# rgrover/cloud-haskell-paxos

Measured on AMD Instinct MI355X. Metric: Paxos instances decided/sec (node), higher is better.
Workload: dtype int32

## Files before the change

### cloud-haskell-paxos_amd/csrc/paxos_ev.h

```cpp
#pragma once
#include <hip/hip_runtime.h>
#include <stdint.h>

#include <type_traits>

#include "../../include/paxos_batch.h"
#include "ev_layouts.h"
#include "paxos_device.h"

namespace pxb {
namespace ev {

#ifndef PXB_EV_SL_RH
#define PXB_EV_SL_RH 1
#endif
#ifndef PXB_EV_LG_RH
#define PXB_EV_LG_RH 0
#endif
#ifndef PXB_EV_STORE_BACK
#define PXB_EV_STORE_BACK 1
#endif
#ifndef PXB_EV_PQ_CAP
#define PXB_EV_PQ_CAP 4
#endif
// ... 93 lines not shown
#else
#define PXB_EV_PROBE(b, c) ((void)0)
#endif

__host__ __device__ __forceinline__ uint32_t u24(uint32_t x) { return x & 0xFFFFFFu; }
template <uint32_t C>
__host__ __device__ __forceinline__ uint32_t mulc(uint32_t x) { return ((C & (C - 1u)) == 0u) ? x * C : u24(x) * C; }
__host__ __device__ __forceinline__ uint32_t ctz32(uint32_t x) { return x ? (uint32_t)__builtin_ctz(x) : 32u; }
__host__ __device__ __forceinline__ uint32_t popc32(uint32_t x) { return (uint32_t)__builtin_popcount(x); }
__host__ __device__ __forceinline__ uint32_t nbits32(uint32_t x) { return x ? 32u - (uint32_t)__builtin_clz(x) : 0u; }

__host__ __device__ __forceinline__ uint32_t window_of(const EvParams& kp, const uint4& w, uint32_t crash_m1) {
  uint32_t c0 = 0, c1 = 0;
  if (w.x <= crash_m1) {
    c0 = mulhi_n(w.y, kp.crash_start_max + 1u);
    c1 = c0 + 1u + mulhi_n(w.z, kp.crash_len_max);
  }
  c0 = c0 < 4096u ? c0 : 4096u;
  c1 = c1 < 4096u ? c1 : 4096u;
  return c0 | (c1 << 16);
}

__host__ __device__ __forceinline__ bool crash_of(const EvParams& kp, uint64_t inst, uint32_t& crash_m1) {
  crash_m1 = kp.crash_m1;
  if (!(kp.cfg & EV_CFG_RANDOMIZE)) return (kp.cfg & EV_CFG_CRASHY) != 0u;
  const uint4 w = philox((uint32_t)inst, (uint32_t)(inst >> 32), 0u, 4u << 24, kp.k0, kp.k1);
  const uint64_t ct = ev_threshold(mulhi_n(w.w, kp.crash_ppm + 1u));
  crash_m1 = (uint32_t)(ct - 1ull);
  return ct != 0ull;
}

__host__ __device__ __forceinline__ uint32_t window_word(const EvParams& kp, uint64_t inst, uint32_t a, bool crashy,
                                                         uint32_t crash_m1) {
  if (!crashy) return 0u;
  return window_of(kp, philox((uint32_t)inst, (uint32_t)(inst >> 32), 0u, (3u << 24) | a, kp.k0, kp.k1), crash_m1);
}

struct EvOut {
  uint32_t res[4];
  uint32_t flags;
  uint32_t steps;
};

struct PhiloxDraws {
  static constexpr bool kPhilox = true;
};
template <class T, class = void>
struct draws_tap : std::false_type {};
template <class T>
struct draws_tap<T, std::void_t<decltype(T::kTap)>> : std::integral_constant<bool, T::kTap> {};

template <int PM, int N, int POOL, int W, bool CMP, class Mem, bool EARLY = true, bool LG = false, bool SL = false,
          int SP = 0, class Src = PhiloxDraws>
struct EvLane : Src {
  using S = Shape<PM, N, POOL, W, CMP, LG, SL, SP>;
  static constexpr bool kEarly = EARLY;
  static constexpr uint32_t A_DEAD = LG ? 24 : 26, A_LEN = LG ? 14 : 27, A_LEN_MAX = LG ? (1u << 18) - 1u : 31;
  using pool_mask_t = typename std::conditional<(POOL > 32), unsigned long long, uint32_t>::type;
  static constexpr uint32_t NLQ = S::NLQ;
  static constexpr uint32_t WM = (uint32_t)W - 1u;
  static constexpr uint32_t QLM = (1u << S::QLB) - 1u, RLM = (1u << S::RLB) - 1u;
  static constexpr uint32_t IM = (1u << S::IB) - 1u;
  static constexpr uint32_t DM = (1u << S::DB) - 1u;

  Mem m;
  uint32_t rk[20];
  uint32_t mode;
  uint32_t gid;
  uint32_t lo, hi;
  uint32_t P, dmax, loss_m1;
  bool lossy;
  static constexpr bool kLossy = !SP;
  int32_t s, last_tick;
  uint32_t acc_mask;
  uint32_t in_mask;
  uint32_t occ;
  static constexpr uint32_t OCC1 = 1u | (1u << W);
  static_assert(2 * W <= 32, "doubled wheel occupancy");
  uint32_t pw0[PM], pw1[PM];
  uint32_t pw2[PM];
  uint32_t skew[PM];
  uint32_t tk_end[PM];
  uint32_t tper;
  uint32_t nsent[PM];
  uint32_t bnext[PM];
  static constexpr bool RPK = PM * S::BR * 4 <= 64;
  using ref_t = typename std::conditional<(PM * S::BR * 4 > 32), unsigned long long, uint32_t>::type;
  ref_t refp;
  uint32_t refc[RPK ? 1 : PM];
  uint32_t accw[N], win[N], accd[N];
  uint32_t accv[LG ? N : 1];
  static constexpr bool RSA = SL && PM == 3;
  static constexpr int NRS = RSA ? N : (NLQ + 3) / 4;
  uint32_t rseqv[SL ? NRS : 1];
  uint32_t pq, pq_len, acur;
#ifdef PXB_EV_CARRY2
  static constexpr bool CARRY2 = SP && EARLY;
#else
  static constexpr bool CARRY2 = false;
#endif
  typename std::conditional<CARRY2, uint32_t, bool>::type pqo;
  uint32_t canon0;
  pool_mask_t pfree;
  uint32_t lflags, rounds, dval, dtick, execs, msgs, canon;
  unsigned long long clog;
  uint32_t clog_len;
  bool bailed;

  __host__ __device__ static constexpr pool_mask_t full_pool() {
    return (POOL == 8 * (int)sizeof(pool_mask_t)) ? ~(pool_mask_t)0
                                                   : (pool_mask_t)((((pool_mask_t)1 << (POOL % (8 * sizeof(pool_mask_t)))) - 1u) << S::POOLB_SHIFT);
  }
  static_assert(POOL + S::POOLB_SHIFT <= 8 * (int)sizeof(pool_mask_t), "pool mask");

  __host__ __device__ static __forceinline__ uint32_t opaque(uint32_t x) {
#if defined(__HIP_DEVICE_COMPILE__)
    __asm__("" : "+v"(x));
#endif
    return x;
  }
  __host__ __device__ static __forceinline__ void opaque_barrier() {
#if defined(__HIP_DEVICE_COMPILE__)
    __asm__ volatile("");
#endif
  }
  template <int I>
  __host__ __device__ static __forceinline__ uint32_t lane_mask(uint32_t onehot) {
#if defined(__HIP_DEVICE_COMPILE__)
    uint32_t r;
    __asm__("v_bfe_i32 %0, %1, %2, 1" : "=v"(r) : "v"(onehot), "i"(I));
    return r;
#else
    return (uint32_t)(((int32_t)(onehot << (31 - I))) >> 31);
#endif
  }
  __host__ __device__ static __forceinline__ uint32_t bfi(uint32_t mk, uint32_t x, uint32_t y) {
#if defined(__HIP_DEVICE_COMPILE__) && defined(PXB_EV_BITOP3_BFI)
    return __builtin_amdgcn_bitop3_b32(mk, x, y, 0xCA);
#elif defined(__HIP_DEVICE_COMPILE__)
    uint32_t r;
    __asm__("v_bfi_b32 %0, %1, %2, %3" : "=v"(r) : "v"(mk), "v"(x), "v"(y));
    return r;
#else
    return (mk & x) | (~mk & y);
#endif
  }
  template <int K, int I = 1>
  __host__ __device__ static __forceinline__ uint32_t get_from(const uint32_t (&v)[K], uint32_t oh, uint32_t r) {
    if constexpr (I < K) return get_from<K, I + 1>(v, oh, bfi(lane_mask<I>(oh), v[I], r));
    else return r;
  }
  template <int K>
  __host__ __device__ static __forceinline__ uint32_t get(const uint32_t (&v)[K], uint32_t q) {
    return get_from<K>(v, 1u << q, v[0]);
  }
  template <int K, int I = 0>
  __host__ __device__ static __forceinline__ void set_from(uint32_t (&v)[K], uint32_t oh, uint32_t x) {
    if constexpr (I < K) {
#if defined(__HIP_DEVICE_COMPILE__)
      __asm__("v_bfi_b32 %0, %1, %2, %0" : "+v"(v[I]) : "v"(lane_mask<I>(oh)), "v"(x));
#else
      v[I] = bfi(lane_mask<I>(oh), x, v[I]);
#endif
      set_from<K, I + 1>(v, oh, x);
    }
  }

  template <int K>
  __host__ __device__ static __forceinline__ void put(uint32_t (&v)[K], uint32_t q, uint32_t x) {
    set_from<K>(v, 1u << q, x);
  }

  __host__ __device__ __forceinline__ uint32_t ref_nib(uint32_t q, uint32_t k) const {
    return RPK ? (uint32_t)(refp >> (4u * (q * (uint32_t)S::BR + k))) & 15u : (get(refc, q) >> (4u * k)) & 15u;
  }
  __host__ __device__ __forceinline__ void ref_add(uint32_t q, uint32_t k, uint32_t d) {
    if constexpr (RPK) refp += (ref_t)(typename std::make_signed<ref_t>::type)(int32_t)d << (4u * (q * (uint32_t)S::BR + k));
    else put(refc, q, get(refc, q) + (d << (4u * k)));
  }

  __host__ __device__ static __forceinline__ uint32_t code_of(uint32_t v) {
    return LG ? (((v >> 12) << 24) | (v & 0xFFFu)) : ((v << 24) | 1u);
  }

  __host__ __device__ static uint32_t w_ticket(uint32_t w0) { return w0 & 0xFFFu; }
  __host__ __device__ static uint32_t w_mr_t(uint32_t w0) { return (w0 >> 12) & 0xFFFu; }
  __host__ __device__ static uint32_t w_acks(uint32_t w0) { return (w0 >> 24) & 15u; }
  __host__ __device__ static uint32_t w_state(uint32_t w0) { return (w0 >> 28) & 3u; }
  __host__ __device__ static uint32_t w_pending(uint32_t w0) { return (w0 >> 30) & 1u; }
  __host__ __device__ static uint32_t w_mr_v(uint32_t w1) { return w1 & 3u; }
  __host__ __device__ static uint32_t w_r2_v(uint32_t w1) { return (w1 >> 2) & 3u; }
  __host__ __device__ static uint32_t w_cmd(uint32_t w1) { return (w1 >> 4) & 3u; }
  __host__ __device__ uint32_t p_ticket(int p) const { return w_ticket(pw0[p]); }
  __host__ __device__ uint32_t p_mr_t(int p) const { return w_mr_t(pw0[p]); }
  __host__ __device__ uint32_t p_acks(int p) const { return w_acks(pw0[p]); }
  __host__ __device__ uint32_t p_state(int p) const { return w_state(pw0[p]); }
  __host__ __device__ uint32_t p_pending(int p) const { return w_pending(pw0[p]); }
  __host__ __device__ uint32_t p_mr_v(int p) const { return w_mr_v(pw1[p]); }
  __host__ __device__ uint32_t p_r2_v(int p) const { return w_r2_v(pw1[p]); }
  __host__ __device__ uint32_t p_cmd(int p) const { return w_cmd(pw1[p]); }

  __host__ __device__ static __forceinline__ uint32_t bring_word(uint32_t q, uint32_t slot) {
    if (PM == 2) return slot;
    return q * (S::BR / 2u) + (slot >> 1);
  }
  __host__ __device__ static __forceinline__ uint32_t bring_half(uint32_t q, uint32_t slot) {
    if (PM == 2) return q;
    return slot & 1u;
  }
  __host__ __device__ __forceinline__ uint32_t rsp_ld(uint32_t Lr) const {
    return S::RH ? m.ldh(S::RSP, Lr) : m.ld(S::RSP + Lr);
  }
  __host__ __device__ __forceinline__ void rsp_st(uint32_t Lr, uint32_t v) const {
    if constexpr (S::RH) m.sth(S::RSP, Lr, v);
    else m.st(S::RSP + Lr, v);
  }

  __host__ __device__ __forceinline__ uint32_t ticks_at(int32_t t) const {
    uint32_t r = 0u;
#pragma unroll
    for (int p = 0; p < PM; ++p) r |= ((uint32_t)p < P && skew[p] == (uint32_t)t) ? (1u << (p * (N + 1))) : 0u;
    return r;
  }

  __host__ __device__ __forceinline__ void enter(int32_t t) {
    s = t;
    pqo = CARRY2 ? pq_len : (pq_len != 0u);
    if constexpr (!SP) canon0 = pqo ? canon : canon - 1u;
    const uint32_t slot = (uint32_t)t & WM;
    uint32_t wq, wi;
    if (S::WW == 1) {
      const uint32_t wv = m.ld(S::WHEEL + slot);
      wq = wv & ((1u << NLQ) - 1u);
      wi = wv >> S::ISH;
    } else {
      wq = m.ld(S::WHEEL + 2u * slot);
      wi = m.ld(S::WHEEL + 2u * slot + 1u);
      m.st(S::WHEEL + 2u * slot + 1u, 0u);
    }
    m.st(S::WHEEL + S::WW * slot, 0u);
    occ &= ~(OCC1 << slot);
    acc_mask = wq;
    uint32_t tk = 0u;
    PXB_EV_PROBE(EVP_TICK_ENTER, t <= last_tick);
    if (!SP && any_lane(t <= last_tick)) {
      opaque_barrier();
      tk = (t <= last_tick) ? ticks_at(t) : 0u;
      if constexpr (LG) {
#pragma unroll
        for (int p = 0; p < PM; ++p)
          skew[p] = (((tk >> (p * (N + 1))) & 1u) && skew[p] < tk_end[p]) ? skew[p] + tper : skew[p];
      }
    }
    in_mask = wi | tk;
#pragma unroll
    for (int p = 0; p < PM; ++p) {
      const uint32_t grp = ((1u << S::IW) - 1u) << (p * S::IW);
      canon += (in_mask & grp) ? 48u : 0u;
    }
  }

  __host__ __device__ __forceinline__ void set_keys(const EvParams& kp) {
#pragma unroll
    for (int r = 0; r < 10; ++r) {
#if defined(PXB_EV_SGPR_KEYS) && defined(__HIP_DEVICE_COMPILE__)
      uint32_t a = kp.k0 + (uint32_t)r * 0x9E3779B9u, b = kp.k1 + (uint32_t)r * 0xBB67AE85u;
      __asm__ volatile("" : "+s"(a));
      __asm__ volatile("" : "+s"(b));
      rk[2 * r] = a;
      rk[2 * r + 1] = b;
#else
      rk[2 * r] = opaque(kp.k0 + (uint32_t)r * 0x9E3779B9u);
      rk[2 * r + 1] = opaque(kp.k1 + (uint32_t)r * 0xBB67AE85u);
#endif
    }
  }
  __host__ __device__ __forceinline__ uint4 draw(uint32_t c2, uint32_t c3) const {
    if constexpr (Src::kPhilox) return philox_rk(lo, hi, c2, c3, rk);
    else return Src::source_draw(lo, hi, c2, c3, rk);
  }

  __host__ __device__ __forceinline__ void init(const EvParams& kp, uint32_t g, const uint32_t* wsrc = nullptr) {
    gid = g;
    if (wsrc) {
      const uint32_t* const row = wsrc + (uint64_t)g * N;
#pragma unroll
      for (int a = 0; a < N; ++a) win[a] = row[a];
    }
    const uint64_t inst = kp.first_instance + g;
    lo = (uint32_t)inst;
    hi = (uint32_t)(inst >> 32);
    P = kp.n_prop;
    dmax = kp.delay_max;
    lossy = (kp.cfg & EV_CFG_LOSSY) != 0u;
    bool crashy = (kp.cfg & EV_CFG_CRASHY) != 0u;
    loss_m1 = kp.loss_m1;
    uint32_t crash_m1 = kp.crash_m1;
    if (kp.cfg & EV_CFG_RANDOMIZE) {
      const uint4 w = draw(0u, 4u << 24);
      P = 1u + mulhi_n(w.x, kp.n_prop);
      const uint64_t lt = ev_threshold(mulhi_n(w.y, kp.loss_ppm + 1u));
      dmax = 1u + mulhi_n(w.z, kp.delay_max);
      const uint64_t ct = ev_threshold(mulhi_n(w.w, kp.crash_ppm + 1u));
      lossy = lt != 0ull;
      loss_m1 = (uint32_t)(lt - 1ull);
      crashy = ct != 0ull;
      crash_m1 = (uint32_t)(ct - 1ull);
    }
    if constexpr (SL && PM < 3) {
      if ((kp.cfg & EV_CFG_RANDOMIZE) && !any_lane(P <= (uint32_t)PM)) {
        bailed = true;
        mode = M_RUN;
        return;
      }
    }
    uint4 wsk = make_uint4(0, 0, 0, 0);
    if (kp.skew_max > 0u) wsk = draw(0u, 2u << 24);
    last_tick = 0;
    tper = kp.tick_period;
#pragma unroll
    for (int p = 0; p < PM; ++p) {
      const uint32_t wp = (p == 0) ? wsk.x : (p == 1) ? wsk.y : wsk.z;
      skew[p] = (kp.skew_max > 0u && (uint32_t)p < P) ? mulhi_n(wp, kp.skew_max + 1u) : 0u;
      tk_end[p] = LG ? skew[p] + (kp.n_ticks - 1u) * kp.tick_period : skew[p];
      const int32_t lt = (int32_t)(((uint32_t)p < P) ? tk_end[p] : 0u);
      last_tick = (lt > last_tick) ? lt : last_tick;
      pw0[p] = pw1[p] = pw2[p] = 0u;
      nsent[p] = bnext[p] = 0u;
      refc[RPK ? 0 : p] = 0u;
      refp = 0u;
    }
    if (!wsrc) {
#pragma unroll
      for (int a = 0; a < N; ++a) win[a] = crashy ? window_of(kp, draw(0u, (3u << 24) | (uint32_t)a), crash_m1) : 0u;
    }
#pragma unroll
    for (int a = 0; a < N; ++a) {
      accw[a] = 0u;
      if constexpr (LG) accv[a] = 0u;
      accd[a] = 0x811C9DC5u;
    }
#pragma unroll
    for (int i = S::REQ; i < S::POOLW; ++i) m.st(i, 0u);
    if constexpr (S::RH) {
#pragma unroll
      for (int i = 0; i < NLQ; ++i) m.sth(S::RSP, i, 1u);
    }
    if constexpr (SL) {
#pragma unroll
      for (int i = 0; i < NRS; ++i) rseqv[i] = 0u;
    }
#pragma unroll
    for (int i = 0; i < W * S::WW; ++i) m.st(S::WHEEL + i, 0u);
    pq = pq_len = acur = 0u;
    pqo = 0;
    pfree = full_pool();
    lflags = rounds = dval = dtick = execs = msgs = canon = 0u;
    clog = 0ull;
    clog_len = 0u;
    occ = 0u;
    bailed = P > (uint32_t)PM;
    mode = M_RUN;
    enter(0);
    if constexpr (SP) {
#pragma unroll
      for (int p = 0; p < PM; ++p) {
        if ((uint32_t)p < P) {
          canon += 48u;
          pw0[p] = 1u | (ROUND1 << 28);
          pw1[p] = ((uint32_t)p + 1u) << 4;
          broadcast((uint32_t)p, ASK, 1u, 0u, true, 1u, false, 0u);
        }
      }
      in_mask = 0u;
    }
  }

  __host__ __device__ __forceinline__ void broadcast(uint32_t q, uint32_t kind0, uint32_t x0, uint32_t z0, bool p0,
                                                     uint32_t x1, bool p1, uint32_t val) {
    rounds += ((p0 & (kind0 == ASK)) ? 1u : 0u) + (p1 ? 1u : 0u);
    const bool ex = p0 & (kind0 == EXECUTE);
    execs += ex ? 1u : 0u;
    const bool first = ex & (dval == 0u);
    dval = first ? val : dval;
    dtick = first ? x0 : dtick;
    const uint32_t slot0 = get(bnext, q), slot1 = (slot0 + 1u) & (S::BR - 1u);
    bailed = bailed | (p0 & (ref_nib(q, slot0) != 0u)) | (p1 & (ref_nib(q, slot1) != 0u));
    PXB_EV_PROBE(EVB_RING, (p0 & (ref_nib(q, slot0) != 0u)) | (p1 & (ref_nib(q, slot1) != 0u)));
    PXB_EV_PROBE(EVP_BCAST, p0);
    if (p0) {
      if constexpr (LG && !PXB_EV_STORE_BACK) {
        m.st(S::BRING + q * S::BR + slot0, x0 | (z0 << 12) | (kind0 << 30));
        if (p1) m.st(S::BRING + q * S::BR + slot1, x1 | (ASK << 30));
      } else if constexpr (!LG && !PXB_EV_STORE_BACK) {
        m.st16h(S::BRING + bring_word(q, slot0), bring_half(q, slot0), x0 | (z0 << 12) | (kind0 << 14));
        if (p1) m.st16h(S::BRING + bring_word(q, slot1), bring_half(q, slot1), x1 | (ASK << 14));
      }
    }
    if constexpr (LG && PXB_EV_STORE_BACK) {
      const uint32_t w0a = S::BRING + q * S::BR + slot0, w1a = S::BRING + q * S::BR + slot1;
      const uint32_t o0 = m.ld(w0a), o1 = m.ld(w1a);
      m.st(w0a, p0 ? x0 | (z0 << 12) | (kind0 << 30) : o0);
      m.st(w1a, p1 ? x1 | (ASK << 30) : o1);
    }
    if constexpr (!LG && PXB_EV_STORE_BACK) {
      const uint32_t w0a = S::BRING + bring_word(q, slot0), h0a = bring_half(q, slot0);
      const uint32_t w1a = S::BRING + bring_word(q, slot1), h1a = bring_half(q, slot1);
      const uint32_t o0 = m.ld16h(w0a, h0a), o1 = m.ld16h(w1a, h1a);
      m.st16h(w0a, h0a, p0 ? x0 | (z0 << 12) | (kind0 << 14) : o0);
      m.st16h(w1a, h1a, p1 ? x1 | (ASK << 14) : o1);
    }
    pq |= (p0 ? ((q << 3) | slot0) << (5u * pq_len) : 0u) | (p1 ? ((q << 3) | slot1) << (5u * pq_len + 5u) : 0u);
    const uint32_t nb = (p0 ? 1u : 0u) + (p1 ? 1u : 0u);
    pq_len += nb;
    put(bnext, q, (slot0 + nb) & (S::BR - 1u));
  }

  __host__ __device__ __forceinline__ bool copy_ready() const { return pq_len != 0u; }
  struct Reply {
    bool snd;
    uint32_t Lr, pw, bit;
    uint32_t z;
  };

  __host__ __device__ __forceinline__ void send_first(const EvParams& kp, const uint4& w, const Reply& rp,
                                                     bool act = true) {
    const bool isR = rp.snd;
    const uint32_t sb = (uint32_t)s - (pqo ? 1u : 0u);
    const bool csnd = act & !isR & (pq_len != 0u);
    const uint32_t ce = pq & 31u;
    const uint32_t cp = ce >> 3, cslot = ce & 7u, ca = acur;
    const uint32_t ck = get(nsent, cp);
    {
      const uint32_t a1 = acur + 1u;
      const bool wrap = csnd & (a1 == (uint32_t)N);
      acur = wrap ? 0u : (csnd ? a1 : acur);
      pq = wrap ? pq >> 5 : pq;
      pq_len -= wrap ? 1u : 0u;
      if constexpr (CARRY2) pqo -= (wrap & (pqo != 0u)) ? 1u : 0u;
      else pqo = pqo & !wrap;
      put(nsent, cp, ck + (wrap ? 1u : 0u));
    }
    const bool snd = isR | csnd;
    PXB_EV_PROBE(EVP_SEND1, snd);
    const bool ok = !(kLossy & lossy & (w.x <= loss_m1));
    const uint32_t d = 1u + mulhi_n(w.y, dmax);
    const bool go = snd & ok;
    const uint32_t base = isR ? (uint32_t)s : sb;
    const uint32_t b4 = base & 15u;
    const uint32_t Lq = mulc<PM>(ca) + cp;
    const bool r2c = S::RCODE & isR & ((rp.pw >> 30) == R2S);
    const uint32_t k2 = (POOL > 32) ? (uint32_t)__builtin_ctzll((unsigned long long)pfree | (1ull << 63))
                                    : ctz32((uint32_t)pfree) & 31u;
    uint32_t due_rel, due4;
    if constexpr (S::RH) {
      const uint32_t wq = m.ld(S::REQ + Lq);
      const uint32_t h = rsp_ld(rp.Lr);
      const uint32_t msb = 31u - (uint32_t)__builtin_clz(h | 1u);
      const uint32_t te = (h >> ((msb - (uint32_t)S::IB) & 31u)) & IM;
      const bool tcode = S::RCODE && te >= S::RCB;
      const uint32_t tp = (m.ld(S::POOLB + ((S::TE_SAFE || !tcode) ? te : 0u)) >> 26) & 15u;
      const uint32_t rtail = tcode ? te & 7u : tp;
      const uint32_t qlen = (wq >> S::QL) & QLM;
      const uint32_t qtail = (wq >> (((uint32_t)S::EB * qlen - (uint32_t)S::DB) & 31u)) & DM;
      const uint32_t nz = isR ? h - 1u : qlen;
      constexpr uint32_t RM = S::RCODE ? 7u : 15u;
      static_assert(!S::RCODE || DM == 7u, "codes on the 4-step wheel");
      const uint32_t rel = ((isR ? rtail : qtail) - b4) & (nz ? (isR ? RM : DM) : 0u);
      due_rel = d > rel ? d : rel;
      due4 = (b4 + due_rel) & 15u;
      const uint32_t pool_out = ((pfree == 0) & !r2c) ? 1u : 0u;
      const uint32_t full = isR ? (h >> (S::IB * S::RC)) | pool_out : qlen >> 2;
      static_assert(S::QC == 4, "request FIFOs of 4");
      bailed = bailed | (go & (full != 0u));
      PXB_EV_PROBE(EVB_RFIFO, go & isR & (h >= (1u << (S::IB * S::RC))));
      PXB_EV_PROBE(EVB_POOL, go & isR & (pfree == 0) & !r2c);
      PXB_EV_PROBE(EVB_QFIFO, go & !isR & (qlen >= (uint32_t)S::QC));
      m.st(pfree ? S::POOLB + k2 : S::REQ + Lq, rp.pw | (due4 << 26));
      if constexpr (LG) {
        const uint32_t zi = pfree ? k2 - 1u : (uint32_t)POOL;
        m.st16h(S::POOLZ + (zi >> 1), zi & 1u, rp.z);
      }
      const uint32_t ent = r2c ? S::RCB + (due4 & 7u) : k2;
      const uint32_t nR = h + ((ent + (1u << S::IB) - 1u) << msb);
      const uint32_t nQ = wq + (1u << S::QL) + ((cslot | ((due4 & DM) << S::SB)) << ((uint32_t)S::EB * qlen));
      m.st(S::REQ + Lq, (go & !isR) ? nQ : wq);
      rsp_st(rp.Lr, (go & isR) ? nR : h);
    } else {
      const uint32_t lw = isR ? S::RSP + rp.Lr : S::REQ + Lq;
      const uint32_t wv = m.ld(lw);
      uint32_t rlen, rtail;
      if constexpr (S::RZ) {
        rlen = (nbits32(wv) + (uint32_t)S::IB - 1u) / (uint32_t)S::IB;
        const uint32_t te = (wv >> ((S::IB * rlen - S::IB) & 31u)) & (isR ? IM : 0u);
        rtail = (m.ld(S::POOLB + te) >> 26) & 15u;
      } else {
        rlen = (wv >> S::RL) & RLM;
        rtail = (wv >> S::RD) & 15u;
      }
      const uint32_t qlen = (wv >> S::QL) & QLM;
      const uint32_t qtail = (wv >> (((uint32_t)S::EB * qlen - (uint32_t)S::DB) & 31u)) & DM;
      const uint32_t len = isR ? rlen : qlen;
      const uint32_t tail = isR ? rtail : qtail;
      const uint32_t lm = isR ? 15u : DM;
      const uint32_t rel = (tail - b4) & (len ? lm : 0u);
      due_rel = d > rel ? d : rel;
      due4 = (b4 + due_rel) & 15u;
      const uint32_t pool_out = ((pfree == 0) & !r2c) ? 1u : 0u;
      const uint32_t rfull = (rlen >= (uint32_t)S::RC) ? 1u : 0u, qfull = (qlen >= (uint32_t)S::QC) ? 1u : 0u;
      const uint32_t full = isR ? rfull | pool_out : qfull;
      bailed = bailed | (go & (full != 0u));
      PXB_EV_PROBE(EVB_RFIFO, go & isR & (len >= (uint32_t)S::RC));
      PXB_EV_PROBE(EVB_POOL, go & isR & (pfree == 0) & !r2c);
      PXB_EV_PROBE(EVB_QFIFO, go & !isR & (len >= (uint32_t)S::QC));
      m.st(pfree ? S::POOLB + k2 : lw, rp.pw | (due4 << 26));
      if constexpr (LG) {
        const uint32_t zi = pfree ? k2 : (uint32_t)POOL;
        m.st16h(S::POOLZ + (zi >> 1), zi & 1u, rp.z);
      }
      const uint32_t ent = r2c ? S::RCB + (due4 & 7u) : k2;
      constexpr int RD = S::RZ ? 0 : S::RD;
      const uint32_t nR = S::RZ ? wv | (ent << ((S::IB * len) & 31u))
                                : ((wv + (1u << S::RL) + (ent << (S::IB * len))) & ~(15u << RD)) | (due4 << RD);
      const uint32_t nQ = wv + (1u << S::QL) + ((cslot | ((due4 & DM) << S::SB)) << ((uint32_t)S::EB * len));
      m.st(lw, go ? (isR ? nR : nQ) : wv);
    }
    pfree &= (go & isR & !r2c) ? ~((pool_mask_t)1 << k2) : ~(pool_mask_t)0;
    ref_add(cp, cslot, (go & !isR) ? 1u : 0u);
    const bool now = EARLY & !isR & (base + due_rel == (uint32_t)s);
    const uint32_t slot = (base + due_rel) & WM;
    m.orw(S::WHEEL + slot * S::WW + ((S::WW == 2 && isR) ? 1u : 0u), (go & !now) ? 1u << (isR ? rp.bit : Lq) : 0u);
    occ |= (go & !now) ? (OCC1 << slot) : 0u;
    acc_mask |= (go & now) ? (1u << Lq) : 0u;
  }

  __host__ __device__ __forceinline__ uint2 copy_ctr() const {
    const uint32_t cp = (pq & 31u) >> 3;
    return make_uint2(get(nsent, cp), (1u << 24) | (cp << 8) | acur);
  }
  __host__ __device__ __forceinline__ void copy_send(const EvParams& kp, bool act, const uint4& w) {
    const uint32_t sb = (uint32_t)s - (pqo ? 1u : 0u);
    const uint32_t s4 = sb & 15u;
    const bool snd = act & (pq_len != 0u);
    PXB_EV_PROBE(EVP_COPY, snd);
    const uint32_t ce = pq & 31u;
    const uint32_t cp = ce >> 3, cslot = ce & 7u, ca = acur;
    const uint32_t ck = get(nsent, cp);
    {
      const uint32_t a1 = acur + 1u;
      const bool wrap = snd & (a1 == (uint32_t)N);
      acur = wrap ? 0u : (snd ? a1 : acur);
      pq = wrap ? pq >> 5 : pq;
      pq_len -= wrap ? 1u : 0u;
      if constexpr (CARRY2) pqo -= (wrap & (pqo != 0u)) ? 1u : 0u;
      else pqo = pqo & !wrap;
      put(nsent, cp, ck + (wrap ? 1u : 0u));
    }
    const bool ok = !(kLossy & lossy & (w.x <= loss_m1));
    const uint32_t d = 1u + mulhi_n(w.y, dmax);
    const bool go = snd & ok;
    const uint32_t Lq = mulc<PM>(ca) + cp;
    const uint32_t wq = m.ld(S::REQ + Lq);
    const uint32_t qlen = (wq >> S::QL) & QLM;
    bailed = bailed | (go & (qlen >= (uint32_t)S::QC));
    PXB_EV_PROBE(EVB_QFIFO, go & (qlen >= (uint32_t)S::QC));
    const uint32_t rel = (((wq >> (((uint32_t)S::EB * qlen - (uint32_t)S::DB) & 31u)) & DM) - s4) & (qlen ? DM : 0u);
    const uint32_t due_rel = d > rel ? d : rel;
    const uint32_t ent = cslot | (((s4 + due_rel) & DM) << S::SB);
    m.st(S::REQ + Lq, go ? wq + (1u << S::QL) + (ent << ((uint32_t)S::EB * qlen)) : wq);
    ref_add(cp, cslot, go ? 1u : 0u);
    const bool now = EARLY & (sb + due_rel == (uint32_t)s);
    const uint32_t slot = (sb + due_rel) & WM;
    m.orw(S::WHEEL + slot * S::WW, (go & !now) ? 1u << Lq : 0u);
    occ |= (go & !now) ? (OCC1 << slot) : 0u;
    acc_mask |= (go & now) ? (1u << Lq) : 0u;
  }

  struct NoFin {
    __host__ __device__ void operator()(const EvOut&) const {}
  };
  template <class Fin = NoFin>
  __host__ __device__ __forceinline__ bool step(const EvParams& kp, EvOut& o, bool act = true, const Fin& fin = Fin()) {
    Reply rp;
    prop_op(kp, act);
    const uint2 c = copy_ctr();
    copy_send(kp, act, draw(c.x, c.y));
    const uint32_t ready = acc_ready_mask();
    const uint4 w0 = acc_op(kp, act, copy_ctr(), rp, ready);
    send_first(kp, w0, rp, act);
    return end_op(kp, o, act, fin);
  }

  __host__ __device__ __forceinline__ bool acc_ready() const { return acc_ready_mask() != 0u; }
  __host__ __device__ __forceinline__ uint32_t acc_ready_mask() const {
#ifdef PXB_EV_OLD_READY
    return (EARLY & (pqo != 0)) ? acc_mask & ((1u << (acur * (uint32_t)PM)) - 1u) : acc_mask;
#else
    const uint32_t cp = (pq & 31u) >> 3;
    const uint32_t upto = (PM == 1) ? ~0u : (PM == 2) ? 0x55555555u | (uint32_t)((int32_t)(pq << 28) >> 31)
                                                      : (cp == 0u ? 0x49249249u : cp == 1u ? 0xDB6DB6DBu : ~0u);
    uint32_t ok = ((1u << (acur * (uint32_t)PM)) - 1u) | upto;
    if constexpr (CARRY2) {
      const uint32_t c2 = (pq >> 8) & 3u;
      const uint32_t upto2 = (PM == 1) ? ~0u : (PM == 2) ? 0x55555555u | (uint32_t)((int32_t)(pq << 23) >> 31)
                                                         : (c2 == 0u ? 0x49249249u : c2 == 1u ? 0xDB6DB6DBu : ~0u);
      ok &= ((uint32_t)pqo > 1u) ? upto2 : ~0u;
    }
    return (EARLY & (pqo != 0)) ? acc_mask & ok : acc_mask;
#endif
  }
  __host__ __device__ __forceinline__ uint4 acc_op(const EvParams& kp, bool act, uint2 cc, Reply& rp,
                                                   uint32_t ready) {
    const uint32_t s4 = (uint32_t)s & 15u;
    const bool acc = act & (ready != 0u);
    PXB_EV_PROBE(EVP_ACC, acc);
    const uint32_t L = acc ? ctz32(ready) : 0u;
    const uint32_t a = L / (uint32_t)PM, p = L - a * (uint32_t)PM;
    const uint32_t wq = m.ld(S::REQ + L);
    const uint32_t kw = SL ? get(rseqv, RSA ? a : L >> 2) : 0u;
    const uint32_t ksh = 8u * (RSA ? p : (L & 3u));
    const uint32_t kr = S::CMP ? (wq >> S::KSH) : SL ? (kw >> ksh) & 0xFFu : m.ld16(S::RSEQ, L);
    const uint32_t len = (wq >> S::QL) & QLM;
    const uint32_t bslot = wq & ((1u << S::SB) - 1u);
    const uint32_t rq2 = ((wq & ((1u << S::QL) - 1u)) >> S::EB) + ((wq & ~((1u << S::QL) - 1u)) - (1u << S::QL));
    const bool keep = (len > 1u) & (((wq >> (S::EB + S::SB)) & DM) == (s4 & DM));
    acc_mask = (acc & !keep) ? (acc_mask & ~(1u << L)) : acc_mask;
    uint32_t kind, x, z;
    if constexpr (LG) {
      const uint32_t w32 = m.ld(S::BRING + p * S::BR + bslot);
      kind = w32 >> 30, x = w32 & 0xFFFu, z = (w32 >> 12) & 0x3FFFu;
    } else {
      const uint32_t w16 = m.ld16h(S::BRING + bring_word(p, bslot), bring_half(p, bslot));
      kind = w16 >> 14, x = w16 & 0xFFFu, z = (w16 >> 12) & 3u;
    }
    ref_add(p, bslot, acc ? ~0u : 0u);
    const uint32_t A = get(accw, a);
    const bool dead = ((A >> A_DEAD) & 1u) != 0u;
    const uint32_t wa = get(win, a);
    const bool isol = ((wa & 0xFFFFu) <= (uint32_t)s) & ((uint32_t)s < (wa >> 16));
    const bool live = acc & !dead & !isol;
    const uint32_t rb = (kind == PROPOSE) ? 12u : 8u;
    canon += acc ? (live ? 2u * rb + 32u : rb) : 0u;
    const uint32_t t_max = A & 0xFFFu;
    const uint32_t V = LG ? get(accv, a) : A;
    const uint32_t val = LG ? V & 0x3FFFu : (A >> 24) & 3u;
    uint32_t log_len = V >> A_LEN;
    const bool is_ask = live & (kind == ASK), is_prop = live & (kind == PROPOSE), is_exec = live & (kind == EXECUTE);
    const bool grant = is_ask & !(t_max >= x);
    const bool accept = is_prop & (x == t_max);
    const bool hit = is_exec & (t_max == x);
    const bool panic = hit & (val == 0u);
    const bool run = hit & (val != 0u);
    const uint32_t rz = grant ? val : 0u;
    lflags |= panic ? (uint32_t)PXB_F_PANIC : 0u;
    PXB_EV_PROBE(EVP_RUN, run);
    if (__builtin_expect(run, 0)) {
      if (log_len >= A_LEN_MAX) bailed = true;
      PXB_EV_PROBE(EVB_LOG, log_len >= A_LEN_MAX);
      put(accd, a, fnv_u32(get(accd, a), code_of(val)));
      if constexpr (LG) {
        const bool trk = log_len < (uint32_t)PXB_LOG_TRACK;
        const uint32_t li = trk ? log_len : (uint32_t)PXB_LOG_TRACK - 1u;
        const bool seen = log_len < clog_len;
        const bool app = trk & !seen;
        uint32_t old;
        if constexpr (S::CLP) {
          const uint32_t b = mulc<14>(li), w = b >> 5, sh = b & 31u;
          const uint32_t w1 = (w + 1u < (uint32_t)S::CLW) ? w + 1u : w;
          const uint32_t lo = m.ld(S::CLOG + w), hi = m.ld(S::CLOG + w1);
          const unsigned long long v = ((unsigned long long)hi << 32) | lo;
          old = (uint32_t)(v >> sh) & 0x3FFFu;
          const unsigned long long nv = app ? (v & ~(0x3FFFull << sh)) | ((unsigned long long)val << sh) : v;
          m.st(S::CLOG + w1, (uint32_t)(nv >> 32));
          m.st(S::CLOG + w, (uint32_t)nv);
        } else {
          const uint32_t cw = S::CLOG + (li >> 1), ch = li & 1u;
          old = m.ld16h(cw, ch);
          m.st16h(cw, ch, app ? val : old);
        }
        lflags |= (trk & seen & (old != val)) ? (uint32_t)PXB_F_LOG_DIVERGENCE : 0u;
        lflags |= trk ? 0u : (uint32_t)PXB_F_LOG_TRUNC;
        clog_len += app ? 1u : 0u;
      } else {
        if (log_len < clog_len) {
          if (((uint32_t)(clog >> (2u * log_len)) & 3u) != val) lflags |= PXB_F_LOG_DIVERGENCE;
        } else {
          clog |= (unsigned long long)val << (2u * log_len);
          clog_len += 1u;
        }
      }
      log_len += 1u;
    }
    uint32_t pw;
    if constexpr (LG) {
      const uint32_t c_gr = (A & ~0xFFFu) | x, c_ac = (A & ~0xFFF000u) | (x << 12);
      const uint32_t c_rn = A & ~0xFFF000u, c_pn = A | (1u << A_DEAD);
      uint32_t An = panic ? c_pn : A;
      An = run ? c_rn : An;
      An = accept ? c_ac : An;
      An = grant ? c_gr : An;
      put(accw, a, An);
      const uint32_t v_ac = (V & ~0x3FFFu) | z, v_rn = (V & ~0x3FFFu) + (1u << A_LEN);
      uint32_t Vn = run ? v_rn : V;
      Vn = accept ? v_ac : Vn;
      put(accv, a, Vn);
      const uint32_t p_gr = x | (A & 0xFFF000u) | (R1OK << 30), p_hv = (A & 0xFFFu) | (HAVE << 30);
      constexpr uint32_t p_ac = R2S << 30;
      pw = accept ? p_ac : p_hv;
      pw = grant ? p_gr : pw;
    } else {
      const uint32_t c_gr = (A & ~0xFFFu) | x, c_ac = (A & 0xFC000FFFu) | (x << 12) | (z << 24);
      const uint32_t c_rn = (A & 0xFC000FFFu) + (1u << 27), c_pn = A | (1u << 26);
      uint32_t An = panic ? c_pn : A;
      An = run ? c_rn : An;
      An = accept ? c_ac : An;
      An = grant ? c_gr : An;
      put(accw, a, An);
      const uint32_t p_gr = x | (A & 0x03FFF000u) | (R1OK << 30), p_hv = (A & 0xFFFu) | (HAVE << 30);
      constexpr uint32_t p_ac = R2S << 30;
      pw = accept ? p_ac : p_hv;
      pw = grant ? p_gr : pw;
    }
    const bool snd1 = live & !is_exec;
    if constexpr (draws_tap<Src>::value) Src::tap_acc(acc, a, p, kind, x, z, dead ? 1u : isol ? 2u : 0u, snd1, pw, rz);
    m.st(S::REQ + L, acc ? rq2 + ((S::CMP && snd1) ? 1u << S::KSH : 0u) : wq);

    const uint4 w1 = draw(snd1 ? kr : cc.x, snd1 ? (1u << 24) | (1u << 16) | (p << 8) | a : cc.y);
    msgs += snd1 ? 1u : 0u;
    bailed = bailed | (snd1 & (kr == (S::CMP ? (1u << S::KB) - 1u : SL ? 0xFFu : 0xFFFFu)));
    PXB_EV_PROBE(EVB_RSEQ, snd1 & (kr == (S::CMP ? (1u << S::KB) - 1u : SL ? 0xFFu : 0xFFFFu)));
    if constexpr (SL) put(rseqv, RSA ? a : L >> 2, kw + (snd1 ? 1u << ksh : 0u));
    else if constexpr (!S::CMP) m.st16(S::RSEQ, L, snd1 ? kr + 1u : kr);
    rp.snd = snd1;
    rp.Lr = p * (uint32_t)N + a;
    rp.pw = pw;
    rp.z = rz;
    rp.bit = S::ISH + (SP ? rp.Lr : mulc<N + 1>(p) + 1u + a);
    return w1;
  }

  __host__ __device__ __forceinline__ bool prop_ready() const { return in_mask != 0u && pq_len + 2u <= PQ_CAP; }
  __host__ __device__ __forceinline__ void prop_op(const EvParams& kp, bool act) {
    const uint32_t s4 = (uint32_t)s & 15u;
    const bool pin = act & (in_mask != 0u) & (pq_len + 2u <= PQ_CAP);
    PXB_EV_PROBE(EVP_PROP, pin);
    {
      const uint32_t j = pin ? ctz32(in_mask) : 0u;
      const uint32_t q = SP ? (j * ((65536u + N - 1u) / N)) >> 16 : j / (uint32_t)(N + 1);
      const uint32_t r = SP ? 1u : j - mulc<N + 1>(q);
      const bool resp = pin & (r != 0u);
      const uint32_t ra = r - 1u;
      const uint32_t Lr = SP ? j : mulc<N>(q) + (resp ? ra : 0u);
      const uint32_t rr = rsp_ld(Lr);
      const uint32_t rlen = (rr >> S::RL) & RLM;
      const uint32_t k = rr & IM, nk = (rr >> S::IB) & IM;
      const bool kc = S::RCODE & (k >= S::RCB), nkc = S::RCODE & (nk >= S::RCB);
      const uint32_t pe0 = m.ld(S::POOLB + ((S::TE_SAFE || !kc) ? k : 0u));
      const uint32_t pn = m.ld(S::POOLB + ((S::TE_SAFE || !nkc) ? nk : 0u));
      const uint32_t pe = kc ? (R2S << 30) : pe0;
      pfree |= (resp & !kc) ? ((pool_mask_t)1 << k) : (pool_mask_t)0;
      const uint32_t popped = S::RZ ? rr >> S::IB
                                    : ((rr & ((1u << S::RL) - 1u)) >> S::IB) + ((rr & ~((1u << S::RL) - 1u)) - (1u << S::RL));
      rsp_st(Lr, resp ? popped : rr);
      const bool nnow = nkc ? ((nk & 7u) == (s4 & 7u)) : (((pn >> 26) & 15u) == s4);
      const bool rkeep = resp & (S::RH ? rr >= (1u << (2 * S::IB)) : S::RZ ? nk != 0u : rlen > 1u) & nnow;
      in_mask = (pin & !rkeep) ? (in_mask & ~(1u << j)) : in_mask;
      const uint32_t rkind = pe >> 30, px = pe & 0xFFFu, py = (pe >> 12) & 0xFFFu;
      const uint32_t kz = k - (uint32_t)S::POOLB_SHIFT;
      const uint32_t pz = LG ? m.ld16h(S::POOLZ + ((kz >> 1) & 31u), kz & 1u) : (pe >> 24) & 3u;
      canon += resp ? 32u >> rkind : 0u;

      const uint32_t w0 = get(pw0, q), w1 = get(pw1, q);
      const uint32_t T = w0 & 0xFFFu, MT = (w0 >> 12) & 0xFFFu, K = (w0 >> 24) & 15u, R = (w0 >> 28) & 3u;
      uint32_t MV, C2, CM, CT = 0u;
      if constexpr (LG) {
        CT = get(pw2, q);
        MV = w1 & 0x3FFFu, C2 = (w1 >> 14) & 0x3FFFu, CM = CT ? (((q + 1u) << 12) | CT) : 0u;
      } else {
        MV = w1 & 3u, C2 = (w1 >> 2) & 3u, CM = (w1 >> 4) & 3u;
      }
      {
        const uint32_t maj = (uint32_t)N >> 1;
        const uint32_t key = (pin ? ((!SP && r == 0u) ? 3u : rkind) : 4u) * 4u + R;
        const bool t_go = !SP && key == 3u * 4u + IDLE;
        const bool h_go = (key - (HAVE * 4u + ROUND1) < 2u) & (px >= T);
        const bool o_go = (key == R1OK * 4u + ROUND1) & (T == px);
        const bool s_go = key == R2S * 4u + ROUND2;
        const bool maj1 = K >= maj;
        const bool o_take = (MV == 0u) | ((pz != 0u) & !(MT >= py));
        const uint32_t mv = o_take ? pz : MV;
        const bool o_maj = o_go & maj1, s_maj = s_go & maj1;
        const uint32_t PDb = w0 & (1u << 30);
        const bool sPD = s_maj & (PDb != 0u);
        const bool ask = t_go | h_go;
        const bool restart = ask | sPD;
        const uint32_t Tn = (h_go ? px : T) + (restart ? 1u : 0u);
        const uint32_t C2n = o_maj ? ((mv == 0u) ? CM : mv) : C2;
        const uint32_t dmt = (py - MT) << 12;
        const uint32_t inc = (1u << 24) + ((o_go & o_take) ? dmt : 0u);
        const uint32_t pdo = (mv != 0u) ? 1u << 30 : 0u;
        const uint32_t c_rs = Tn | (ROUND1 << 28) | PDb, c_om = T | (ROUND2 << 28) | pdo;
        const uint32_t c_sd = w0 & 0xFFFFFFu, c_in = w0 + inc;
        uint32_t w0n = (o_go | s_go) ? c_in : w0;
        w0n = s_maj ? c_sd : w0n;
        w0n = o_maj ? c_om : w0n;
        w0n = restart ? c_rs : w0n;
        constexpr uint32_t MVM = LG ? 0x3FFFu : 3u, C2S = LG ? 14u : 2u;
        const uint32_t tick_cm = (SP || LG) ? 0u : ((q + 1u) << 4);
        const uint32_t c1_rs = (!LG && t_go) ? (w1 & 0xCu) | tick_cm : w1 & ~MVM;
        const uint32_t c1_om = (LG ? 0u : (w1 & 0x30u)) | (C2n << C2S);
        const uint32_t c1_ok = (w1 & ~MVM) | mv, c1_sd = LG ? w1 : w1 & 0xFu;
        uint32_t w1n = s_maj ? c1_sd : w1;
        w1n = o_go ? c1_ok : w1n;
        w1n = o_maj ? c1_om : w1n;
        w1n = restart ? c1_rs : w1n;
        put(pw0, q, w0n);
        put(pw1, q, w1n);
        if constexpr (LG) put(pw2, q, t_go ? Tn : (s_maj & (PDb == 0u)) ? 0u : CT);
        const uint32_t k0o = ask ? ASK : o_maj ? PROPOSE : s_maj ? EXECUTE : NONE;
        if constexpr (draws_tap<Src>::value) Src::tap_prop(pin, q, r, rkind, px, py, pz, k0o, ask ? Tn : T, Tn, C2n, sPD);
        broadcast(q, k0o, ask ? Tn : T, C2n, k0o != NONE, Tn, sPD, C2n);
      }
    }
  }

  __host__ __device__ __forceinline__ bool end_ready(const EvParams& kp) const {
    const bool carry = EARLY & (pq_len <= (CARRY2 ? 2u : 1u)) & !pqo & ((uint32_t)s + 1u < kp.step_cap);
    return (acc_mask == 0u) & (in_mask == 0u) & ((pq_len == 0u) | carry);
  }
  template <class Fin = NoFin>
  __host__ __device__ __forceinline__ bool end_op(const EvParams& kp, EvOut& o, bool act, const Fin& fin = Fin()) {
    if (act && end_ready(kp)) {
      PXB_EV_PROBE(EVP_END, true);
      const bool quiet = (pq_len == 0u) & (occ == 0u) & (SP || s >= last_tick);
      const bool back = EARLY & !SP & (canon == canon0);
      const uint32_t s1 = (uint32_t)s + 1u;
      const uint32_t rot = (occ >> (s1 & WM)) & ((1u << W) - 1u);
      uint32_t nx = ((occ != 0u) & (pq_len == 0u)) ? s1 + ctz32(rot) : (pq_len ? s1 : 0xFFFFu);
      PXB_EV_PROBE(EVP_TICK_END, s < last_tick);
      if (!SP && any_lane(s < last_tick)) {
        opaque_barrier();
#pragma unroll
        for (int q = 0; q < PM; ++q) nx = ((skew[q] > (uint32_t)s) & (skew[q] < nx)) ? skew[q] : nx;
      }
      const bool capped = !quiet & (nx >= kp.step_cap);
      PXB_EV_PROBE(EVP_FIN, quiet | capped);
      if (__builtin_expect(quiet | capped, 0)) {
        s = capped ? (int32_t)kp.step_cap - 1 : (back ? s - 1 : s);
        finish(capped, o);
        fin(o);
        return true;
      }
      enter((int32_t)nx);
    }
    return false;
  }

  __host__ __device__ __forceinline__ uint32_t msgs_sent() const {
    uint32_t b = 0u;
#pragma unroll
    for (int p = 0; p < PM; ++p) b += nsent[p];
    return msgs + b * (uint32_t)N;
  }

  __host__ __device__ __forceinline__ void finish(bool capped, EvOut& o) {
    const uint32_t steps = (uint32_t)s + 1u;
    uint32_t f = lflags | (capped ? (uint32_t)PXB_F_STEP_CAP : 0u) | (dval ? 0u : (uint32_t)PXB_F_UNDECIDED);
#pragma unroll
    for (int p = 0; p < PM; ++p)
      f |= (!capped && (uint32_t)p < P && p_state(p) != IDLE) ? (uint32_t)PXB_F_STUCK : 0u;
    canon += 16u + 4u * (uint32_t)N;
    o.res[0] = dval ? code_of(dval) : 0u;
    o.res[1] = dval ? dtick : 0u;
    o.res[2] = rounds;
    o.res[3] = (f & 0xFFu) | (steps << 16);
    o.flags = f;
    o.steps = steps;
    mode = M_IDLE;
  }

  __host__ __device__ uint32_t links_in_flight() const {
    uint32_t n = 0u;
    for (uint32_t L = 0; L < NLQ; ++L) {
      const uint32_t rw = rsp_ld(L);
      n += ((m.ld(S::REQ + L) >> S::QL) & QLM)
           + (S::RH ? (nbits32(rw) - 1u) / (uint32_t)S::IB
              : S::RZ ? (nbits32(rw) + (uint32_t)S::IB - 1u) / (uint32_t)S::IB : (rw >> S::RL) & RLM);
    }
    return n;
  }

  __host__ __device__ static uint32_t w_log_len(uint32_t V) { return V >> A_LEN; }
  __host__ __device__ uint32_t log_len_of(int a) const { return w_log_len(LG ? accv[LG ? a : 0] : accw[a]); }
  __host__ __device__ static uint32_t w_digest(uint32_t D, uint32_t len) {
    if constexpr (LG) {
      return fnv_u32(D, len);
    } else {
      constexpr uint32_t P = 0x01000193u, P2 = P * P, P4 = P2 * P2;
      static_assert(A_LEN_MAX < 256, "one-byte log length");
      return (D ^ len) * P4;
    }
  }
  __host__ __device__ uint32_t digest_of(int a) const { return w_digest(accd[a], log_len_of(a)); }
  __host__ __device__ static void w_record(uint32_t A, uint32_t V, uint32_t r[4]) {
    const uint32_t val = LG ? V & 0x3FFFu : (A >> 24) & 3u;
    r[0] = A & 0xFFFu;
    r[1] = (A >> 12) & 0xFFFu;
    r[2] = val ? code_of(val) : 0u;
    r[3] = w_log_len(V) | (((A >> A_DEAD) & 1u) << 31);
  }
  __host__ __device__ void record_of(int a, uint32_t r[4]) const { w_record(accw[a], LG ? accv[LG ? a : 0] : accw[a], r); }
};

__host__ inline EvParams make_params(const pxb_config* c) {
  EvParams p{};
  p.first_instance = c->first_instance;
  p.k0 = (uint32_t)c->seed;
  p.k1 = (uint32_t)(c->seed >> 32);
  p.n_prop = c->n_proposers;
  p.delay_max = c->delay_max;
  p.loss_ppm = c->loss_ppm;
  p.crash_ppm = c->crash_ppm;
  p.crash_len_max = c->crash_len_max;
  p.crash_start_max = c->crash_start_max;
  p.skew_max = c->skew_max;
  p.step_cap = c->step_cap;
  p.n_ticks = c->n_ticks > 1 ? c->n_ticks : 1u;
  p.tick_period = c->n_ticks > 1 ? c->tick_period : 1u;
  const uint64_t lt = ev_threshold(c->loss_ppm), ct = ev_threshold(c->crash_ppm);
  p.cfg = ((c->flags & PXB_CFG_RANDOMIZE) ? EV_CFG_RANDOMIZE : 0u) | (lt ? EV_CFG_LOSSY : 0u) | (ct ? EV_CFG_CRASHY : 0u);
  if ((c->flags & PXB_CFG_RANDOMIZE) || lt || c->delay_max > 1) p.cfg |= EV_CFG_DRAWS;
  p.loss_m1 = (uint32_t)(lt - 1ull);
  p.crash_m1 = (uint32_t)(ct - 1ull);
  return p;
}

}
}
```

### cloud-haskell-paxos_amd/csrc/script_core.h

```cpp
#pragma once
#include <stdint.h>

#include "../../include/paxos_batch.h"
#include "paxos_ev.h"

namespace pxb {
namespace ev {

constexpr uint32_t SCR_HDR = 16u;
constexpr uint32_t SCR_KEEP8 = 0xFFu, SCR_KEEP16 = 0xFFFFu;

__host__ __device__ inline uint64_t script_links_off(uint32_t N) { return SCR_HDR + 4ull * N; }
__host__ __device__ inline uint64_t script_links_bytes(uint32_t P, uint32_t N, uint32_t depth) {
  return 2ull * P * N * depth;
}
__host__ __device__ inline uint64_t script_stride(uint32_t P, uint32_t N, uint32_t depth) {
  return (script_links_off(N) + script_links_bytes(P, N, depth) + 7ull) & ~7ull;
}
__host__ __device__ __forceinline__ uint32_t script_ld16(const uint8_t* r, uint32_t off) {
  return (uint32_t)r[off] | ((uint32_t)r[off + 1u] << 8);
}

struct ScriptInst {
  uint32_t P, dmax, loss_m1, crash_m1;
// ... 78 lines not shown
    if ((c3 >> 24) == 2u) return make_uint4(s_skew[0] << 16, s_skew[1] << 16, s_skew[2] << 16, 0u);
    const uint32_t dirn = (c3 >> 16) & 0xFFu, p = (c3 >> 8) & 0xFFu, a = c3 & 0xFFu, k = c2;
    const bool in = ((c3 >> 24) == 1u) & (dirn < 2u) & (p < s_P) & (a < s_N) & (k < s_depth);
    uint32_t b = SCR_KEEP8;
    if (in) b = byte_at(((uint64_t)((dirn * s_P + p) * s_N + a)) * s_depth + k);
    const uint4 w = philox_rk(lo, hi, c2, c3, rk);
    const bool keep = b == SCR_KEEP8;
    const bool lost = keep ? s_lossy & (w.x <= s_loss_m1) : b == 0u;
    uint32_t d = keep ? 1u + mulhi_n(w.y, s_dmax) : (b < s_dclamp ? b : s_dclamp);
    d = d < 1u ? 1u : (d > 15u ? 15u : d);
    return make_uint4(lost ? 0u : 1u, (d - 1u) << 28, 0u, 0u);
  }
  struct RowByte {
    const uint8_t* links;
    __host__ __device__ __forceinline__ uint32_t operator()(uint64_t i) const { return links[i]; }
  };
  __host__ __device__ __forceinline__ uint4 source_draw(uint32_t lo, uint32_t hi, uint32_t c2, uint32_t c3,
                                                        const uint32_t (&rk)[20]) const {
    return source_draw_over(lo, hi, c2, c3, rk, RowByte{s_links});
  }
};

struct ScriptNoNeutral {
  __host__ __device__ __forceinline__ bool operator()(uint32_t) const { return false; }
};
template <class Lane, class Neutral>
__host__ __device__ __forceinline__ uint32_t script_begin_sel(Lane& L, const EvParams& kp, uint32_t depth,
                                                              const uint8_t* row, const Neutral& neutral) {
  constexpr uint32_t P = Lane::S::PM, N = Lane::S::N;
  static_assert(!Lane::S::SP && !Lane::S::CMP && !Lane::S::SL, "the generic shape");
  const uint32_t lo = script_ld16(row, 0) | (script_ld16(row, 2) << 16);
  const uint32_t hi = script_ld16(row, 4) | (script_ld16(row, 6) << 16);
  const uint32_t np = row[8];
  if ((np > P) | (row[9] != 0u)) return PXB_SCRIPT_BAD;
  const ScriptInst si = script_inst(kp, lo, hi);
  ScriptDraws& D = L;
  D.s_links = row + script_links_off(N);
  D.s_depth = depth;
  D.s_P = P;
  D.s_N = N;
  D.s_dclamp = kp.delay_max;
  D.s_dmax = si.dmax;
  D.s_loss_m1 = si.loss_m1;
  D.s_lossy = si.lossy;
#pragma unroll
  for (uint32_t p = 0; p < 3u; ++p) {
    const uint32_t v = script_ld16(row, 10u + 2u * p);
    D.s_skew[p] = neutral(p) ? 0u : v == SCR_KEEP16 ? script_skew(kp, lo, hi, p) : v;
  }
  EvParams pl = kp;
  pl.first_instance = (uint64_t)lo | ((uint64_t)hi << 32);
  pl.cfg = EV_CFG_LOSSY | EV_CFG_DRAWS;
  pl.n_prop = np ? np : si.P;
  pl.delay_max = 16u;
  pl.loss_m1 = 0u;
  pl.skew_max = 0xFFFFu;
  L.init(pl, 0u);
#pragma unroll
  for (uint32_t a = 0; a < N; ++a) {
    uint32_t c0 = script_ld16(row, SCR_HDR + 4u * a), c1 = script_ld16(row, SCR_HDR + 4u * a + 2u);
    uint32_t wv;
    if ((c0 == SCR_KEEP16) & (c1 == SCR_KEEP16)) {
      wv = script_window(kp, si, lo, hi, a);
    } else {
      c0 = c0 < 4096u ? c0 : 4096u;
      c1 = c1 < 4096u ? c1 : 4096u;
      wv = c0 >= c1 ? 0u : c0 | (c1 << 16);
    }
    L.win[a] = neutral(3u + a) ? 0u : wv;
  }
  return PXB_TRACE_OK;
}
template <class Lane>
__host__ __device__ __forceinline__ uint32_t script_begin(Lane& L, const EvParams& kp, uint32_t depth,
                                                          const uint8_t* row) {
  return script_begin_sel(L, kp, depth, row, ScriptNoNeutral{});
}

template <class Lane>
__host__ __device__ __forceinline__ void script_sent(const Lane& L, uint16_t* out) {
  constexpr uint32_t P = Lane::S::PM, N = Lane::S::N;
  for (uint32_t p = 0; p < P; ++p)
    for (uint32_t a = 0; a < N; ++a) {
      out[p * N + a] = (uint16_t)(p < L.P ? L.nsent[p] : 0u);
      out[(P + p) * N + a] = (uint16_t)(p < L.P ? L.m.ld16(Lane::S::RSEQ, a * P + p) : 0u);
    }
}

}
}
```

Measured before the change: 70.73 million.

## Pack per-proposer send counters and ring cursors into shared registers

For shapes with at most two proposers, the per-proposer nsent and bnext arrays are packed into two 32-bit words (16-bit fields) so they can be updated by shifted adds instead of indexed select chains. The pending-queue append is rewritten to build both entries at once and mask by count, mask-clearing is turned into XOR, and opaque() barriers are placed on a few loads to steer the compiler. The aim is fewer VGPRs and fewer select instructions per lane. The risk is that bnext is no longer masked on wrap, since the field is only masked when read, which relies on a 16-bit field overflowing cleanly.

```diff
diff --git a/cloud-haskell-paxos_amd/csrc/paxos_ev.h b/cloud-haskell-paxos_amd/csrc/paxos_ev.h
--- a/cloud-haskell-paxos_amd/csrc/paxos_ev.h
+++ b/cloud-haskell-paxos_amd/csrc/paxos_ev.h
@@ -199,8 +199,10 @@
   uint32_t skew[PM];
   uint32_t tk_end[PM];
   uint32_t tper;
-  uint32_t nsent[PM];
-  uint32_t bnext[PM];
+  static constexpr bool CPK = PM <= 2;
+  uint32_t nsp, bcp;
+  uint32_t nsent[CPK ? 1 : PM];
+  uint32_t bnext[CPK ? 1 : PM];
   static constexpr bool RPK = PM * S::BR * 4 <= 64;
   using ref_t = typename std::conditional<(PM * S::BR * 4 > 32), unsigned long long, uint32_t>::type;
   ref_t refp;
@@ -294,6 +296,24 @@
   __host__ __device__ __forceinline__ void ref_add(uint32_t q, uint32_t k, uint32_t d) {
     if constexpr (RPK) refp += (ref_t)(typename std::make_signed<ref_t>::type)(int32_t)d << (4u * (q * (uint32_t)S::BR + k));
     else put(refc, q, get(refc, q) + (d << (4u * k)));
+  }
+
+  __host__ __device__ static __forceinline__ uint32_t fld_sh(uint32_t q) { return PM == 1 ? 0u : q << 4; }
+  __host__ __device__ __forceinline__ uint32_t nsent_of(uint32_t q) const {
+    if constexpr (CPK) return PM == 1 ? nsp : (nsp >> fld_sh(q)) & 0xFFFFu;
+    else return get(nsent, q);
+  }
+  __host__ __device__ __forceinline__ void nsent_add(uint32_t q, uint32_t ck, uint32_t d) {
+    if constexpr (CPK) nsp += d << fld_sh(q);
+    else put(nsent, q, ck + d);
+  }
+  __host__ __device__ __forceinline__ uint32_t bslot_of(uint32_t q) const {
+    if constexpr (CPK) return (bcp >> fld_sh(q)) & (S::BR - 1u);
+    else return get(bnext, q);
+  }
+  __host__ __device__ __forceinline__ void bslot_add(uint32_t q, uint32_t slot0, uint32_t nb) {
+    if constexpr (CPK) bcp += nb << fld_sh(q);
+    else put(bnext, q, (slot0 + nb) & (S::BR - 1u));
   }
 
   __host__ __device__ static __forceinline__ uint32_t code_of(uint32_t v) {
@@ -443,7 +463,8 @@
       const int32_t lt = (int32_t)(((uint32_t)p < P) ? tk_end[p] : 0u);
       last_tick = (lt > last_tick) ? lt : last_tick;
       pw0[p] = pw1[p] = pw2[p] = 0u;
-      nsent[p] = bnext[p] = 0u;
+      nsent[CPK ? 0 : p] = bnext[CPK ? 0 : p] = 0u;
+      nsp = bcp = 0u;
       refc[RPK ? 0 : p] = 0u;
       refp = 0u;
     }
@@ -501,7 +522,7 @@
     const bool first = ex & (dval == 0u);
     dval = first ? val : dval;
     dtick = first ? x0 : dtick;
-    const uint32_t slot0 = get(bnext, q), slot1 = (slot0 + 1u) & (S::BR - 1u);
+    const uint32_t slot0 = CPK ? opaque(bslot_of(q)) : bslot_of(q), slot1 = (slot0 + 1u) & (S::BR - 1u);
     bailed = bailed | (p0 & (ref_nib(q, slot0) != 0u)) | (p1 & (ref_nib(q, slot1) != 0u));
     PXB_EV_PROBE(EVB_RING, (p0 & (ref_nib(q, slot0) != 0u)) | (p1 & (ref_nib(q, slot1) != 0u)));
     PXB_EV_PROBE(EVP_BCAST, p0);
@@ -527,10 +548,11 @@
       m.st16h(w0a, h0a, p0 ? x0 | (z0 << 12) | (kind0 << 14) : o0);
       m.st16h(w1a, h1a, p1 ? x1 | (ASK << 14) : o1);
     }
-    pq |= (p0 ? ((q << 3) | slot0) << (5u * pq_len) : 0u) | (p1 ? ((q << 3) | slot1) << (5u * pq_len + 5u) : 0u);
     const uint32_t nb = (p0 ? 1u : 0u) + (p1 ? 1u : 0u);
+    const uint32_t ent2 = u24(q) * 0x108u + (slot0 | (slot1 << 5));
+    pq |= (ent2 & ((1u << (5u * nb)) - 1u)) << (5u * pq_len);
     pq_len += nb;
-    put(bnext, q, (slot0 + nb) & (S::BR - 1u));
+    bslot_add(q, slot0, nb);
   }
 
   __host__ __device__ __forceinline__ bool copy_ready() const { return pq_len != 0u; }
@@ -547,7 +569,7 @@
     const bool csnd = act & !isR & (pq_len != 0u);
     const uint32_t ce = pq & 31u;
     const uint32_t cp = ce >> 3, cslot = ce & 7u, ca = acur;
-    const uint32_t ck = get(nsent, cp);
+    const uint32_t ck = nsent_of(cp);
     {
       const uint32_t a1 = acur + 1u;
       const bool wrap = csnd & (a1 == (uint32_t)N);
@@ -556,7 +578,7 @@
       pq_len -= wrap ? 1u : 0u;
       if constexpr (CARRY2) pqo -= (wrap & (pqo != 0u)) ? 1u : 0u;
       else pqo = pqo & !wrap;
-      put(nsent, cp, ck + (wrap ? 1u : 0u));
+      nsent_add(cp, ck, wrap ? 1u : 0u);
     }
     const bool snd = isR | csnd;
     PXB_EV_PROBE(EVP_SEND1, snd);
@@ -653,7 +675,7 @@
 
   __host__ __device__ __forceinline__ uint2 copy_ctr() const {
     const uint32_t cp = (pq & 31u) >> 3;
-    return make_uint2(get(nsent, cp), (1u << 24) | (cp << 8) | acur);
+    return make_uint2(nsent_of(cp), (1u << 24) | (cp << 8) | acur);
   }
   __host__ __device__ __forceinline__ void copy_send(const EvParams& kp, bool act, const uint4& w) {
     const uint32_t sb = (uint32_t)s - (pqo ? 1u : 0u);
@@ -662,7 +684,7 @@
     PXB_EV_PROBE(EVP_COPY, snd);
     const uint32_t ce = pq & 31u;
     const uint32_t cp = ce >> 3, cslot = ce & 7u, ca = acur;
-    const uint32_t ck = get(nsent, cp);
+    const uint32_t ck = nsent_of(cp);
     {
       const uint32_t a1 = acur + 1u;
       const bool wrap = snd & (a1 == (uint32_t)N);
@@ -671,7 +693,7 @@
       pq_len -= wrap ? 1u : 0u;
       if constexpr (CARRY2) pqo -= (wrap & (pqo != 0u)) ? 1u : 0u;
       else pqo = pqo & !wrap;
-      put(nsent, cp, ck + (wrap ? 1u : 0u));
+      nsent_add(cp, ck, wrap ? 1u : 0u);
     }
     const bool ok = !(kLossy & lossy & (w.x <= loss_m1));
     const uint32_t d = 1u + mulhi_n(w.y, dmax);
@@ -741,7 +763,7 @@
     const uint32_t bslot = wq & ((1u << S::SB) - 1u);
     const uint32_t rq2 = ((wq & ((1u << S::QL) - 1u)) >> S::EB) + ((wq & ~((1u << S::QL) - 1u)) - (1u << S::QL));
     const bool keep = (len > 1u) & (((wq >> (S::EB + S::SB)) & DM) == (s4 & DM));
-    acc_mask = (acc & !keep) ? (acc_mask & ~(1u << L)) : acc_mask;
+    acc_mask ^= ((acc & !keep) ? 1u : 0u) << L;
     uint32_t kind, x, z;
     if constexpr (LG) {
       const uint32_t w32 = m.ld(S::BRING + p * S::BR + bslot);
@@ -859,16 +881,16 @@
   __host__ __device__ __forceinline__ bool prop_ready() const { return in_mask != 0u && pq_len + 2u <= PQ_CAP; }
   __host__ __device__ __forceinline__ void prop_op(const EvParams& kp, bool act) {
     const uint32_t s4 = (uint32_t)s & 15u;
-    const bool pin = act & (in_mask != 0u) & (pq_len + 2u <= PQ_CAP);
+    const bool pin = act & (in_mask != 0u) & (pq_len <= PQ_CAP - 2u);
     PXB_EV_PROBE(EVP_PROP, pin);
     {
-      const uint32_t j = pin ? ctz32(in_mask) : 0u;
+      const uint32_t j = pin ? (uint32_t)__builtin_ctz(in_mask) : 0u;
       const uint32_t q = SP ? (j * ((65536u + N - 1u) / N)) >> 16 : j / (uint32_t)(N + 1);
       const uint32_t r = SP ? 1u : j - mulc<N + 1>(q);
       const bool resp = pin & (r != 0u);
       const uint32_t ra = r - 1u;
       const uint32_t Lr = SP ? j : mulc<N>(q) + (resp ? ra : 0u);
-      const uint32_t rr = rsp_ld(Lr);
+      const uint32_t rr = S::RH ? opaque(rsp_ld(Lr)) : rsp_ld(Lr);
       const uint32_t rlen = (rr >> S::RL) & RLM;
       const uint32_t k = rr & IM, nk = (rr >> S::IB) & IM;
       const bool kc = S::RCODE & (k >= S::RCB), nkc = S::RCODE & (nk >= S::RCB);
@@ -881,7 +903,7 @@
       rsp_st(Lr, resp ? popped : rr);
       const bool nnow = nkc ? ((nk & 7u) == (s4 & 7u)) : (((pn >> 26) & 15u) == s4);
       const bool rkeep = resp & (S::RH ? rr >= (1u << (2 * S::IB)) : S::RZ ? nk != 0u : rlen > 1u) & nnow;
-      in_mask = (pin & !rkeep) ? (in_mask & ~(1u << j)) : in_mask;
+      in_mask ^= ((pin & !rkeep) ? 1u : 0u) << j;
       const uint32_t rkind = pe >> 30, px = pe & 0xFFFu, py = (pe >> 12) & 0xFFFu;
       const uint32_t kz = k - (uint32_t)S::POOLB_SHIFT;
       const uint32_t pz = LG ? m.ld16h(S::POOLZ + ((kz >> 1) & 31u), kz & 1u) : (pe >> 24) & 3u;
@@ -906,9 +928,9 @@
         const bool maj1 = K >= maj;
         const bool o_take = (MV == 0u) | ((pz != 0u) & !(MT >= py));
         const uint32_t mv = o_take ? pz : MV;
-        const bool o_maj = o_go & maj1, s_maj = s_go & maj1;
+        const bool o_maj = o_go && maj1, s_maj = s_go && maj1;
         const uint32_t PDb = w0 & (1u << 30);
-        const bool sPD = s_maj & (PDb != 0u);
+        const bool sPD = s_maj & (opaque(PDb) != 0u);
         const bool ask = t_go | h_go;
         const bool restart = ask | sPD;
         const uint32_t Tn = (h_go ? px : T) + (restart ? 1u : 0u);
@@ -976,7 +998,7 @@
   __host__ __device__ __forceinline__ uint32_t msgs_sent() const {
     uint32_t b = 0u;
 #pragma unroll
-    for (int p = 0; p < PM; ++p) b += nsent[p];
+    for (int p = 0; p < PM; ++p) b += nsent_of((uint32_t)p);
     return msgs + b * (uint32_t)N;
   }
 
diff --git a/cloud-haskell-paxos_amd/csrc/script_core.h b/cloud-haskell-paxos_amd/csrc/script_core.h
--- a/cloud-haskell-paxos_amd/csrc/script_core.h
+++ b/cloud-haskell-paxos_amd/csrc/script_core.h
@@ -184,7 +184,7 @@
   constexpr uint32_t P = Lane::S::PM, N = Lane::S::N;
   for (uint32_t p = 0; p < P; ++p)
     for (uint32_t a = 0; a < N; ++a) {
-      out[p * N + a] = (uint16_t)(p < L.P ? L.nsent[p] : 0u);
+      out[p * N + a] = (uint16_t)(p < L.P ? L.nsent_of(p) : 0u);
       out[(P + p) * N + a] = (uint16_t)(p < L.P ? L.m.ld16(Lane::S::RSEQ, a * P + p) : 0u);
     }
 }
```

After: 74.99 million, median of 6. +6.0%, better.
